# cristicbz/rust-doom

Hardware: NVIDIA H100
Metric: frames/sec at 1920x1080 (palette-index bit-exact) (higher is better)
Workload: dtype u8

## Files before the change

rust-doom_b200/csrc/b2d_kernels.cu:

```cuda
#include "b2d_kernels.cuh"

namespace b2d {

namespace {

constexpr unsigned kFull = 0xFFFFFFFFu;

constexpr int kMaskWords = 128;
constexpr int kStackDepth = 128;

constexpr uint32_t kVisBit = 1u << 25, kSolidBit = 1u << 24;
__device__ __forceinline__ uint32_t pack_range(int lo, int hi, uint32_t bits) {
    return (uint32_t)lo | ((uint32_t)hi << 12) | bits;
}
__device__ __forceinline__ int range_lo(uint32_t r) { return (int)(r & 0xFFFu); }
__device__ __forceinline__ int range_hi(uint32_t r) { return (int)((r >> 12) & 0xFFFu); }

__device__ __forceinline__ uint32_t word_bits(int w, int lo, int hi) {
    int a = max(lo, w * 32), b = min(hi, w * 32 + 31);
    if (a > b) return 0u;
    uint32_t m = 0xFFFFFFFFu >> (31 - (b - w * 32));
    return m & (0xFFFFFFFFu << (a - w * 32));
}

// ... 409 lines not shown
    uint8_t *p8 = c.fb + (size_t)y0 * Wc;
    uint32_t *p32 = kRgba ? c.rgba + (size_t)y0 * Wc : nullptr;
#pragma unroll 2
    for (int y = y0; y < y1; y++, p8 += Wc, p32 += Wc) {
        const uint32_t r = sc.skyrow[y];
        put_px<kRgba>(c, p8, p32, y >= ya && y < yb, __ldg(px + (inter ? (r >> 2) * w4 + (r & 3u) : r * T.w)));
    }
}

template <bool kRgba, int kW>
__device__ __forceinline__ void draw_plane_warp(const RasterCtx &c, const FrameConst &fc, const View &vw,
                                                int ya, int yb, int32_t h, int32_t flat, int lightb,
                                                bool visible) {
    const DeviceScene &sc = *c.sc;
    if (!__any_sync(kFull, ya < yb)) return;
    if (!visible) { fill_void_warp<kRgba, kW>(c, ya, yb); return; }
    if (flat == kFlatSky) { draw_sky_warp<kRgba, kW>(c, ya, yb); return; }
    if (flat < 0 || flat >= sc.nflats) { fill_void_warp<kRgba, kW>(c, ya, yb); return; }
    const uint64_t px_hi = reinterpret_cast<uint64_t>(sc.lit_flats) & 0xFFFFFFFF00000000ull;
    const uint32_t habs = plane_habs(h, fc.pose.z);
    bool act = ya < yb;
    int y0 = __reduce_min_sync(kFull, act ? ya : 0x7FFFFFFF);
    int y1 = __reduce_max_sync(kFull, act ? yb : 0);
    const int full_lo = __reduce_max_sync(kFull, act ? ya : 0x7FFFFFFF);
    const int full_hi = __reduce_min_sync(kFull, act ? yb : 0);
    const int Wc = kW ? kW : c.W;
    uint8_t *p8 = c.fb + (size_t)y0 * Wc;
    uint32_t *p32 = kRgba ? c.rgba + (size_t)y0 * Wc : nullptr;
    const uint32_t bu = (uint32_t)fc.pose.x << 10, bv = (uint32_t)fc.pose.y << 10;
    const uint32_t ax = (uint32_t)c.dir.ax, ay = (uint32_t)c.dir.ay;
    for (int yc = y0; yc < y1; yc += 32) {
        int yy = yc + c.lane;
        if (yy < y1) {
            const PlaneRow pr = plane_row(habs, sc.yslope[yy]);
            c.rowz[c.lane] = make_uint2(pr.z8q, (sc.lit_flat_stride >> 6) * (uint32_t)light_row(lightb, pr.z8) + 64u * (uint32_t)flat);
        }
        __syncwarp();
        const int rows = min(32, y1 - yc);
        int j = 0;
        for (; j + kBatch <= rows; j += kBatch, p8 += (size_t)kBatch * Wc, p32 += (size_t)kBatch * Wc) {
            uint32_t v[kBatch];
#pragma unroll
            for (int k = 0; k < kBatch; k++) {
                const uint2 rz = c.rowz[j + k];
                v[k] = __ldg(reinterpret_cast<const uint8_t *>(px_hi | flat_offset(rz.y, bu + rz.x * ax, bv + rz.x * ay)));
            }
            const int y = yc + j;
            store_batch<kRgba, kW>(c, p8, p32, v, y, ya, yb, y >= full_lo && y + kBatch <= full_hi);
        }
        for (; j < rows; j++, p8 += Wc, p32 += Wc) {
            const uint2 rz = c.rowz[j];
            const int y = yc + j;
            put_px<kRgba>(c, p8, p32, y >= ya && y < yb,
                          __ldg(reinterpret_cast<const uint8_t *>(px_hi | flat_offset(rz.y, bu + rz.x * ax, bv + rz.x * ay))));
        }
        __syncwarp();
    }
}

template <bool kRgba, int kW, int R>
__device__ __forceinline__ void wall_fast_loop(const RasterCtx &c, const uint8_t *plq, uint32_t w4, uint32_t nq, uint32_t q,
                                               uint32_t acc, uint32_t ts29, int y0, int y1, int ya, int yb,
                                               int full_lo, int full_hi) {
    const int Wc = kW ? kW : c.W;
    uint8_t *p8 = c.fb + (size_t)y0 * Wc;
    uint32_t *p32 = kRgba ? c.rgba + (size_t)y0 * Wc : nullptr;
    asm("" : "+l"(plq));
#pragma unroll 1
    for (int y = y0; y < y1; y += R, p8 += (size_t)R * Wc, p32 += (size_t)R * Wc) {
        const uint32_t q1 = q + 1u == nq ? 0u : q + 1u;
        const uint32_t w0 = __ldg(reinterpret_cast<const uint32_t *>(plq + (size_t)q * w4));
        const uint32_t w1 = __ldg(reinterpret_cast<const uint32_t *>(plq + (size_t)q1 * w4));
        if (y >= full_lo && y + R <= full_hi) {
#pragma unroll
            for (int k = 0; k < R; k++) {
                uint32_t v = pick_byte(w0, w1, wall_sel(acc, ts29, (uint32_t)k));
                if (kRgba) v &= 0xFFu;
                put_px<kRgba>(c, p8 + (size_t)k * Wc, kRgba ? p32 + (size_t)k * Wc : nullptr, true, v);
            }
        } else {
            const uint32_t m = row_mask(y, ya, yb, R);
#pragma unroll
            for (int k = 0; k < R; k++) {
                uint32_t v = pick_byte(w0, w1, wall_sel(acc, ts29, (uint32_t)k));
                if (kRgba) v &= 0xFFu;
                put_px<kRgba>(c, p8 + (size_t)k * Wc, kRgba ? p32 + (size_t)k * Wc : nullptr, (m >> k) & 1u, v);
            }
        }
        wall_advance(acc, q, ts29, (uint32_t)R, nq);
    }
}

template <bool kRgba, int kW>
__device__ __forceinline__ void draw_wall_warp(const RasterCtx &c, const FrameConst &fc, int ya, int yb,
                                               int32_t tex, int32_t tA, int32_t hA, int32_t ucol,
                                               int32_t iscale, int row) {
    const DeviceScene &sc = *c.sc;
    if (!__any_sync(kFull, ya < yb)) return;
    if (tex < 0 || tex >= sc.ntex) { fill_void_warp<kRgba, kW>(c, ya, yb); return; }
    const TexRec T = sc.tex[tex];
    bool act = ya < yb;
    const uint32_t col = (uint32_t)floormod32(ucol, (int32_t)T.w);
    const uint8_t *pl = sc.lit_texels + (size_t)row * sc.lit_texel_stride + T.texel_off;
    const uint32_t tstep = (uint32_t)(iscale >> 4);
    int y0 = __reduce_min_sync(kFull, act ? ya : 0x7FFFFFFF);
    int y1 = __reduce_max_sync(kFull, act ? yb : 0);
    const int full_lo = __reduce_max_sync(kFull, act ? ya : 0x7FFFFFFF);
    const int full_hi = __reduce_min_sync(kFull, act ? yb : 0);
    uint32_t t = (uint32_t)wall_tbase(tA, hA, fc.pose.z, c.H, iscale) + (uint32_t)y0 * tstep;
    const int Wc = kW ? kW : c.W;
    uint8_t *p8 = c.fb + (size_t)y0 * Wc;
    uint32_t *p32 = kRgba ? c.rgba + (size_t)y0 * Wc : nullptr;
    if (tex_interleaved(T) && T.h >= 8u) {
        const uint32_t ts = act ? tstep : 0u;
        const bool f16 = __all_sync(kFull, ts <= kWallFast16);
        if (f16 || __all_sync(kFull, ts <= kWallFast8)) {
            const uint32_t tt = act ? t : 0u;
            const uint32_t r0 = wall_row((int32_t)tt, T.h, T.hmagic, T.hbias);
            const uint8_t *plq = pl + 4u * col;
            if (f16) wall_fast_loop<kRgba, kW, 16>(c, plq, 4u * T.w, T.h >> 2, r0 >> 2, wall_acc29(tt, r0), ts << 13, y0, y1, ya, yb, full_lo, full_hi);
            else wall_fast_loop<kRgba, kW, 8>(c, plq, 4u * T.w, T.h >> 2, r0 >> 2, wall_acc29(tt, r0), ts << 13, y0, y1, ya, yb, full_lo, full_hi);
            return;
        }
    }
    if (tex_interleaved(T)) {
        const uint32_t colb = 4u * col, w4 = 4u * T.w;
        for (int y = y0; y < y1; y += kBatch, p8 += (size_t)kBatch * Wc, p32 += (size_t)kBatch * Wc, t += (uint32_t)kBatch * tstep) {
            const uint32_t r0 = wall_row((int32_t)t, T.h, T.hmagic, T.hbias);
            const uint32_t acc = wall_acc(t, r0);
            const uint32_t b7 = (acc + 7u * tstep) >> 16;
            uint32_t v[kBatch];
            if (__all_sync(kFull, b7 < 8u)) {
                const uint32_t q0 = r0 >> 2, q1 = next_quad(q0, T.h);
                const uint32_t w0 = __ldg(reinterpret_cast<const uint32_t *>(pl + (q0 * w4 + colb)));
                const uint32_t w1 = __ldg(reinterpret_cast<const uint32_t *>(pl + (q1 * w4 + colb)));
#pragma unroll
                for (int k = 0; k < kBatch; k++) {
                    v[k] = pick_byte(w0, w1, (acc + (uint32_t)k * tstep) >> 16);
                    if (kRgba) v[k] &= 0xFFu;
                }
            } else {
                const uint32_t t4 = t + 4u * tstep;
                const uint32_t r4 = wall_row((int32_t)t4, T.h, T.hmagic, T.hbias);
                const uint32_t acc4 = wall_acc(t4, r4);
                if (__all_sync(kFull, ((acc + 3u * tstep) >> 16) < 8u && ((acc4 + 3u * tstep) >> 16) < 8u)) {
                    const uint32_t q0 = r0 >> 2, q4 = r4 >> 2;
                    const uint32_t a0 = __ldg(reinterpret_cast<const uint32_t *>(pl + (q0 * w4 + colb)));
                    const uint32_t a1 = __ldg(reinterpret_cast<const uint32_t *>(pl + (next_quad(q0, T.h) * w4 + colb)));
                    const uint32_t b0 = __ldg(reinterpret_cast<const uint32_t *>(pl + (q4 * w4 + colb)));
                    const uint32_t b1 = __ldg(reinterpret_cast<const uint32_t *>(pl + (next_quad(q4, T.h) * w4 + colb)));
#pragma unroll
                    for (int k = 0; k < 4; k++) {
                        v[k] = pick_byte(a0, a1, (acc + (uint32_t)k * tstep) >> 16);
                        v[k + 4] = pick_byte(b0, b1, (acc4 + (uint32_t)k * tstep) >> 16);
                        if (kRgba) { v[k] &= 0xFFu; v[k + 4] &= 0xFFu; }
                    }
                } else {
#pragma unroll
                    for (int k = 0; k < kBatch; k++) {
                        const uint32_t rk = wall_row((int32_t)(t + (uint32_t)k * tstep), T.h, T.hmagic, T.hbias);
                        v[k] = __ldg(pl + ((rk >> 2) * w4 + colb + (rk & 3u)));
                    }
                }
            }
            store_batch<kRgba, kW>(c, p8, p32, v, y, ya, yb, y >= full_lo && y + kBatch <= full_hi);
        }
    } else {
        const uint8_t *px = pl + col;
#pragma unroll 1
        for (int y = y0; y < y1; y++, p8 += Wc, p32 += Wc, t += tstep)
            put_px<kRgba>(c, p8, p32, y >= ya && y < yb, __ldg(px + wall_row((int32_t)t, T.h, T.hmagic, T.hbias) * T.w));
    }
}

__device__ __forceinline__ uint32_t *masked_entry(const DeviceScene &sc, const uint32_t *chunks, int e) {
    return sc.masked_list + ((size_t)chunks[e / kMaskedChunk] * kMaskedChunk + (size_t)(e % kMaskedChunk)) * 33u;
}
__device__ __forceinline__ uint32_t *masked_push(const DeviceScene &sc, uint32_t *chunks, int &mcount, int lane) {
    bool ok = mcount < sc.masked_cap;
    if (ok && mcount % kMaskedChunk == 0) {
        uint32_t id = 0;
        if (lane == 0) id = atomicAdd(sc.masked_counter, 1u);
        id = __shfl_sync(kFull, id, 0);
        ok = id < sc.masked_chunks;
        if (ok && lane == 0) chunks[mcount / kMaskedChunk] = id;
        __syncwarp();
    }
    if (!ok) {
        if (lane == 0) atomicOr(sc.status_flag, kStatusMaskedFull);
        return nullptr;
    }
    return masked_entry(sc, chunks, mcount++);
}

template <bool kRgba, int kW, bool kStates, bool kLevels>
__device__ __noinline__ void masked_pass(const DeviceScene &sc, const View &vw, int32_t pose_z, uint8_t *fb,
                                         uint32_t *rgba, uint32_t pal_s, int x, int lane,
                                         const SegFrame *wl, const uint32_t *chunks, int count) {
    RasterCtx c;
    c.sc = &sc; c.pal_s = pal_s; c.fb = fb; c.rgba = rgba;
    c.W = vw.W; c.H = vw.H; c.x = x; c.lane = lane;
    const int Wc = kW ? kW : c.W;
    for (int e = count - 1; e >= 0; e--) {
        const uint32_t *ml = masked_entry(sc, chunks, e);
        const uint32_t k = ml[0];
        const uint32_t packed = ml[1 + c.lane];
        int ya = (int)(packed & 0xFFFFu), yb = (int)(packed >> 16);
        const SegFrame sf = wl[k];
        int32_t tex, tA, hA, ucol = 0, iscale = 1, row = 0;
        if (is_sprite_entry(sf)) {
            SpriteFrame sp;
            const SpriteRec P = sc.sprites[entry_sprite(sf, sp)];
            if (P.tex < 0 || P.tex >= sc.ntex) continue;
            const int32_t sw = (int32_t)sc.tex[P.tex].w, sh = (int32_t)sc.tex[P.tex].h;
            const int64_t scale = sprite_scale(vw, sp.cz);
            int32_t z8;
            scale_depth(vw, scale, iscale, z8);
            row = light_row_sprite(P.light, z8);
            tex = P.tex; tA = 0; hA = P.low + sh;
            if (ya < yb) {
                clip_rows(P.low + sh, P.low, row_scale(scale), pose_z, c.H, ya, yb);
                ucol = sprite_column(sp, vw, c.x, sw);
            }
        } else {
            const SegRec S = sc.segs[sf.seg];
            if (S.mid < 0 || S.mid >= sc.nmids) continue;
            const MidRec M = sc.mids[S.mid];
            tex = M.tex; tA = M.t_high; hA = M.high;
            ColumnEval ce = {0u, 1, 1, 0};
            if (ya < yb && column_eval(sf, vw, c.x, ce)) {
                clip_rows(M.high, M.low, ce.scale, pose_z, c.H, ya, yb);
                ucol = wall_column(S.uoff, S.len_q12, ce.s24);
                iscale = ce.iscale;
                row = light_row(S.light, ce.z8);
            } else {
                ya = yb = 0;
            }
        }
        if (tex < 0 || tex >= sc.ntex) continue;
        const TexRec T = sc.tex[tex];
        const bool act = ya < yb;
        int y0 = __reduce_min_sync(kFull, act ? ya : 0x7FFFFFFF);
        int y1 = __reduce_max_sync(kFull, act ? yb : 0);
        if (y0 >= y1) continue;
        const uint32_t col = (uint32_t)floormod32(ucol, (int32_t)T.w);
        const bool inter = tex_interleaved(T);
        const bool has_mask = T.mask_off != 0xFFFFFFFFu;
        const uint8_t *pl = sc.lit_texels + (size_t)row * sc.lit_texel_stride + T.texel_off;
        const uint8_t *pm = sc.lit_texels + (size_t)32 * sc.lit_texel_stride + T.texel_off;
        const uint32_t tstep = (uint32_t)(iscale >> 4);
        uint32_t t = (uint32_t)wall_tbase(tA, hA, pose_z, c.H, iscale) + (uint32_t)y0 * tstep;
        uint8_t *p8 = c.fb + (size_t)y0 * Wc;
        uint32_t *p32 = kRgba ? c.rgba + (size_t)y0 * Wc : nullptr;
        const uint32_t len = act ? (uint32_t)(yb - ya) : 0u;
        if (inter) {
            const uint32_t colb = 4u * col, w4 = 4u * T.w;
#pragma unroll 1
            for (int y = y0; y < y1; y += kBatch, p8 += (size_t)kBatch * Wc, p32 += (size_t)kBatch * Wc, t += (uint32_t)kBatch * tstep) {
                const uint32_t r0 = wall_row((int32_t)t, T.h, T.hmagic, T.hbias);
                const uint32_t acc = wall_acc(t, r0);
                const uint32_t d = (uint32_t)(y - ya);
                uint32_t v[kBatch], o[kBatch];
                if (__all_sync(kFull, ((acc + 7u * tstep) >> 16) < 8u)) {
                    const uint32_t o0 = (r0 >> 2) * w4 + colb, o1 = next_quad(r0 >> 2, T.h) * w4 + colb;
                    const uint32_t w0 = __ldg(reinterpret_cast<const uint32_t *>(pl + o0));
                    const uint32_t w1 = __ldg(reinterpret_cast<const uint32_t *>(pl + o1));
                    uint32_t m0 = 0x01010101u, m1 = 0x01010101u;
                    if (has_mask) {
                        m0 = __ldg(reinterpret_cast<const uint32_t *>(pm + o0));
                        m1 = __ldg(reinterpret_cast<const uint32_t *>(pm + o1));
                    }
#pragma unroll
                    for (int k = 0; k < kBatch; k++) {
                        const uint32_t bk = (acc + (uint32_t)k * tstep) >> 16;
                        v[k] = pick_byte(w0, w1, bk) & 0xFFu;
                        o[k] = pick_byte(m0, m1, bk) & 0xFFu;
                    }
                } else {
#pragma unroll
                    for (int k = 0; k < kBatch; k++) {
                        const uint32_t rk = wall_row((int32_t)(t + (uint32_t)k * tstep), T.h, T.hmagic, T.hbias);
                        const uint32_t off = (rk >> 2) * w4 + colb + (rk & 3u);
                        v[k] = __ldg(pl + off);
                        o[k] = has_mask ? (uint32_t)__ldg(pm + off) : 1u;
                    }
                }
#pragma unroll
                for (int k = 0; k < kBatch; k++)
                    put_px<kRgba>(c, p8 + (size_t)k * Wc, kRgba ? p32 + (size_t)k * Wc : nullptr, d + (uint32_t)k < len && o[k] != 0u, v[k]);
            }
        } else {
#pragma unroll 1
            for (int y = y0; y < y1; y++, p8 += Wc, p32 += Wc, t += tstep) {
                const uint32_t off = wall_row((int32_t)t, T.h, T.hmagic, T.hbias) * T.w + col;
                const bool on = (uint32_t)(y - ya) < len && (!has_mask || __ldg(pm + off) != 0);
                put_px<kRgba>(c, p8, p32, on, __ldg(pl + off));
            }
        }
    }
}

constexpr int kRasterWarps = 8;

template <bool kRgba, int kW, bool kMasked, bool kStates, bool kLevels>
__global__ void __launch_bounds__(32 * kRasterWarps, 16 / kRasterWarps)
b2d_raster_kernel(const __grid_constant__ DeviceScene sc, const __grid_constant__ View vw, const FrameConst *__restrict__ frames,
                  const SegFrame *__restrict__ work, int stride, int n, int strips,
                  uint8_t *__restrict__ index_fb, uint32_t *__restrict__ rgba_fb, const __grid_constant__ StateTables st,
                  const __grid_constant__ LevelTables lt) {
    __shared__ uint32_t s_pal[kRgba ? (kLevels ? 256 * kRasterWarps : 256) : 1];
    __shared__ uint2 s_rowz[kRasterWarps][32];
    __shared__ uint32_t s_chunks[kRasterWarps][kMasked ? kMaskedCapMax / kMaskedChunk : 1];
    if (kRgba && !kLevels) {
        for (int i = threadIdx.x; i < 256; i += blockDim.x) s_pal[i] = sc.palette[i];
        __syncthreads();
    }

    const int lane = threadIdx.x & 31;
    const long long gw = (long long)blockIdx.x * (blockDim.x >> 5) + (threadIdx.x >> 5);
    if (gw >= (long long)n * strips) return;
    const int frame = (int)(gw / strips), strip = (int)(gw % strips);
    const int W = kW ? kW : vw.W, H = vw.H;
    const int x0 = strip * 32, x = x0 + lane;
    const bool inside = x < W;

    const FrameConst fc = frames[frame];
    const DeviceScene *scp = &sc;
    if constexpr (kStates && !kLevels) {
        __shared__ DeviceScene s_sc[kRasterWarps];
        DeviceScene *d = &s_sc[threadIdx.x >> 5];
        const uint32_t *src = reinterpret_cast<const uint32_t *>(&sc);
        uint32_t *dst = reinterpret_cast<uint32_t *>(d);
        for (int i = lane; i < (int)(sizeof(DeviceScene) / 4); i += 32) dst[i] = src[i];
        __syncwarp();
        if (lane == 0) {
            const uint8_t *tb = st.base + (size_t)(uint32_t)fc.pad[0] * st.slot_bytes;
            d->tex = reinterpret_cast<const TexRec *>(tb);
            d->sectors = reinterpret_cast<const SectorRec *>(tb + st.off_sectors);
            d->segs = reinterpret_cast<const SegRec *>(tb + st.off_segs);
            d->sprites = reinterpret_cast<const SpriteRec *>(tb + st.off_sprites);
            d->mids = reinterpret_cast<const MidRec *>(tb + st.off_mids);
        }
        __syncwarp();
        scp = d;
    }
    if constexpr (kLevels) {
        __shared__ DeviceScene s_lv[kRasterWarps];
        DeviceScene *d = &s_lv[threadIdx.x >> 5];
        const DeviceScene *lsrc = lt.scenes + (uint32_t)fc.pad[1];
        const uint32_t *src = reinterpret_cast<const uint32_t *>(lsrc);
        uint32_t *dst = reinterpret_cast<uint32_t *>(d);
        for (int i = lane; i < (int)(sizeof(DeviceScene) / 4); i += 32) dst[i] = src[i];
        if (kRgba) {
            const uint32_t *pal = lsrc->palette;
            for (int i = lane; i < 256; i += 32) s_pal[256 * (threadIdx.x >> 5) + i] = pal[i];
        }
        __syncwarp();
        if constexpr (kStates) {
            if (lane == 0) {
                const TableSet t = lt.sets[(uint32_t)fc.pad[0]];
                d->tex = t.tex; d->sectors = t.sectors; d->segs = t.segs; d->sprites = t.sprites; d->mids = t.mids;
            }
            __syncwarp();
        }
        scp = d;
    }
    const DeviceScene &ts = *scp;
    const DeviceScene &ls = kLevels ? ts : sc;
    RasterCtx c;
    c.sc = &ts;
    c.pal_s = (uint32_t)__cvta_generic_to_shared(kLevels ? s_pal + 256 * (threadIdx.x >> 5) : s_pal);
    c.rowz = s_rowz[threadIdx.x >> 5];
    c.dir = plane_dir(fc, vw, inside ? x : 0, ls.invF);
    c.fb = index_fb + (size_t)frame * W * H + (inside ? x : 0);
    c.rgba = kRgba ? rgba_fb + (size_t)frame * W * H + (inside ? x : 0) : nullptr;
    c.W = W; c.H = H; c.x = x; c.lane = lane;
    c.skycol = 0;
    if (ls.sky_tex >= 0 && inside) c.skycol = umulhi32(sky_u32(x, vw, fc.pose.angle), ts.tex[ls.sky_tex].w);

    int ct = 0, cb = inside ? H : 0;
    uint32_t *chunks = s_chunks[threadIdx.x >> 5];
    asm("" : "+l"(chunks));
    const bool defer = kMasked && ls.masked_list != nullptr;
    int mcount = 0;
    const SegFrame *wl = work + (size_t)frame * stride;
    const int count = fc.count;
    bool done = false;

    for (int k0 = 0; k0 < count && !done; k0 += 32) {
        int k = k0 + lane;
        bool overlap = false;
        if (k < count) {
            int xlo = wl[k].xlo, xhi = wl[k].xhi;
            overlap = xhi >= x0 && xlo <= x0 + 31;
        }
        unsigned m = __ballot_sync(kFull, overlap);
        while (m) {
            int j = __ffs(m) - 1;
            m &= m - 1;
            if (!__any_sync(kFull, ct < cb)) { done = true; break; }
            const SegFrame sf = wl[k0 + j];
            bool in = inside && ct < cb && x >= sf.xlo && x <= sf.xhi;
            if (!__any_sync(kFull, in)) continue;
            if (is_sprite_entry(sf)) {
                if (defer) {
                    uint32_t *ml = masked_push(ls, chunks, mcount, lane);
                    if (ml) {
                        if (lane == 0) ml[0] = (uint32_t)(k0 + j);
                        ml[1 + lane] = in ? ((uint32_t)ct | ((uint32_t)cb << 16)) : 0u;
                    }
                }
                continue;
            }
            ColumnEval ce = {0u, 1, 1, 0};
            bool ok = in && column_eval(sf, vw, x, ce);
            if (!__any_sync(kFull, ok)) continue;

            const SegRec S = ts.segs[sf.seg];
            const SectorRec SF = ts.sectors[S.front];
            const int32_t fcl = SF.ceil, ffl = SF.floor;
            const bool two = S.flags & kSegTwoSided;
            const bool ceil_vis = plane_visible(true, fcl, SF.ceil_flat == kFlatSky, fc.pose.z);
            const bool floor_vis = plane_visible(false, ffl, SF.floor_flat == kFlatSky, fc.pose.z);

            WallRows wr = {ct, ct, ct, ct};
            int yend = ct, row = 0;
            int32_t ucol = 0;
            if (ok) {
                row = light_row(S.light, ce.z8);
                ucol = wall_column(S.uoff, S.len_q12, ce.s24);
                wr = wall_rows(fcl, ffl, two, S.otop, S.obot, ce.scale, fc.pose.z, H, ct, cb);
                yend = cb;
            }
#pragma unroll 1
            for (int pz = 0; pz < 2; pz++) {
                const bool top = pz == 0;
                draw_plane_warp<kRgba, kW>(c, fc, vw, ok ? (top ? ct : wr.y4) : 0, ok ? (top ? wr.y1 : yend) : 0,
                                                    top ? fcl : ffl, top ? SF.ceil_flat : SF.floor_flat, SF.light,
                                                    top ? ceil_vis : floor_vis);
            }
#pragma unroll 1
            for (int pw = 0; pw < 2; pw++) {
                const bool upper = pw == 0;
                if (!wall_piece(upper, two, fcl, ffl, S.otop, S.obot)) continue;
                draw_wall_warp<kRgba, kW>(c, fc, ok ? (upper ? wr.y1 : wr.y3) : 0, ok ? (upper ? wr.y2 : wr.y4) : 0,
                                                   upper ? S.texA : S.texB, upper ? S.tA : S.tB, upper ? S.hA : S.hB,
                                                   ucol, ce.iscale, row);
            }
            if (ok) wall_window(two, wr, H, ct, cb);
            if (defer && two && S.mid >= 0) {
                const bool keep = ok && wr.y2 < wr.y3;
                if (__any_sync(kFull, keep)) {
                    uint32_t *ml = masked_push(ls, chunks, mcount, lane);
                    if (ml) {
                        if (lane == 0) ml[0] = (uint32_t)(k0 + j);
                        ml[1 + lane] = keep ? ((uint32_t)wr.y2 | ((uint32_t)wr.y3 << 16)) : 0u;
                    }
                }
            }
        }
    }
    fill_void_warp<kRgba, kW>(c, inside ? ct : 0, inside ? cb : 0);
    if (kMasked && mcount > 0) {
        __syncwarp();
        masked_pass<kRgba, kW, kStates, kLevels>(ts, vw, fc.pose.z, c.fb, c.rgba, c.pal_s, x, lane, wl, chunks, mcount);
    }
}

__global__ void __launch_bounds__(256)
b2d_palette_kernel(const uint32_t *__restrict__ palette, const uint8_t *__restrict__ index,
                   uint32_t *__restrict__ rgba, size_t n_pixels) {
    __shared__ uint32_t s_pal[256];
    s_pal[threadIdx.x] = palette[threadIdx.x];
    __syncthreads();
    const bool aligned = ((reinterpret_cast<uintptr_t>(index) | reinterpret_cast<uintptr_t>(rgba)) & 15) == 0;
    const size_t nvec = aligned ? n_pixels / 16 : 0;
    const size_t stride = (size_t)gridDim.x * blockDim.x;
    for (size_t i = (size_t)blockIdx.x * blockDim.x + threadIdx.x; i < nvec; i += stride) {
        uint4 in = __ldcs(reinterpret_cast<const uint4 *>(index) + i);
        uint32_t wds[4] = {in.x, in.y, in.z, in.w};
        uint4 *out = reinterpret_cast<uint4 *>(rgba) + 4 * i;
#pragma unroll
        for (int q = 0; q < 4; q++) {
            uint4 o;
            o.x = s_pal[wds[q] & 0xFF];
            o.y = s_pal[(wds[q] >> 8) & 0xFF];
            o.z = s_pal[(wds[q] >> 16) & 0xFF];
            o.w = s_pal[wds[q] >> 24];
            __stcs(out + q, o);
        }
    }
    for (size_t p = nvec * 16 + (size_t)blockIdx.x * blockDim.x + threadIdx.x; p < n_pixels; p += stride)
        rgba[p] = s_pal[index[p]];
}

__global__ void __launch_bounds__(256)
b2d_palette_levels_kernel(const uint32_t *__restrict__ palettes, const uint32_t *__restrict__ tables,
                          const uint8_t *__restrict__ index, uint32_t *__restrict__ rgba, size_t npix, int parts) {
    __shared__ uint32_t s_pal[256];
    const size_t frame = blockIdx.x / parts;
    const int part = blockIdx.x % parts;
    s_pal[threadIdx.x] = palettes[(size_t)tables[frame] * 256 + threadIdx.x];
    __syncthreads();
    const uint8_t *in = index + frame * npix;
    uint32_t *out = rgba + frame * npix;
    const bool aligned = npix % 16 == 0 && ((reinterpret_cast<uintptr_t>(index) | reinterpret_cast<uintptr_t>(rgba)) & 15) == 0;
    const size_t n = aligned ? npix / 16 : npix;
    const size_t per = (n + parts - 1) / parts, lo = (size_t)part * per, hi = lo + per < n ? lo + per : n;
    if (aligned) {
        for (size_t i = lo + threadIdx.x; i < hi; i += blockDim.x) {
            const uint4 q = __ldcs(reinterpret_cast<const uint4 *>(in) + i);
            const uint32_t wds[4] = {q.x, q.y, q.z, q.w};
            uint4 *o4 = reinterpret_cast<uint4 *>(out) + 4 * i;
#pragma unroll
            for (int k = 0; k < 4; k++) {
                uint4 o;
                o.x = s_pal[wds[k] & 0xFF];
                o.y = s_pal[(wds[k] >> 8) & 0xFF];
                o.z = s_pal[(wds[k] >> 16) & 0xFF];
                o.w = s_pal[wds[k] >> 24];
                __stcs(o4 + k, o);
            }
        }
    } else {
        for (size_t p = lo + threadIdx.x; p < hi; p += blockDim.x) out[p] = s_pal[in[p]];
    }
}

constexpr int kResolveRgba = 0, kResolveRgb = 1, kResolvePlanar = 2, kResolveGray = 3;

template <int N>
__device__ __forceinline__ void store_run(uint8_t *dst, const uint32_t (&w)[(N + 3) / 4]) {
    const uintptr_t a = reinterpret_cast<uintptr_t>(dst);
    if constexpr (N % 16 == 0) {
        if ((a & 15) == 0) {
#pragma unroll
            for (int q = 0; q < N / 16; q++) __stcs(reinterpret_cast<uint4 *>(dst) + q, make_uint4(w[4 * q], w[4 * q + 1], w[4 * q + 2], w[4 * q + 3]));
            return;
        }
    }
    if constexpr (N % 8 == 0) {
        if ((a & 7) == 0) {
#pragma unroll
            for (int q = 0; q < N / 8; q++) __stcs(reinterpret_cast<uint2 *>(dst) + q, make_uint2(w[2 * q], w[2 * q + 1]));
            return;
        }
    }
    if constexpr (N % 4 == 0) {
        if ((a & 3) == 0) {
#pragma unroll
            for (int q = 0; q < N / 4; q++) __stcs(reinterpret_cast<unsigned int *>(dst) + q, w[q]);
            return;
        }
    }
    if constexpr (N % 2 == 0) {
        if ((a & 1) == 0) {
#pragma unroll
            for (int q = 0; q < N / 2; q++) reinterpret_cast<uint16_t *>(dst)[q] = (uint16_t)(w[q / 2] >> (16 * (q % 2)));
            return;
        }
    }
#pragma unroll
    for (int b = 0; b < N; b++) dst[b] = (uint8_t)(w[b / 4] >> (8 * (b % 4)));
}

template <int K, int FMT, int P>
__device__ __forceinline__ void resolve_emit(uint8_t *o, size_t opix, int OW, int y, int x0, const uint32_t (&acc0)[P],
                                             const uint32_t (&acc1)[P]) {
    constexpr uint32_t kk = K * K, half = K * K / 2;
    const size_t at = (size_t)y * OW + x0;
    if constexpr (FMT == kResolveGray) {
        uint32_t w[(P + 3) / 4] = {};
#pragma unroll
        for (int p = 0; p < P; p++) w[p / 4] |= ((acc0[p] + half) / kk) << (8 * (p % 4));
        store_run<P>(o + at, w);
    } else {
        uint32_t r[P], g[P], b[P];
#pragma unroll
        for (int p = 0; p < P; p++) {
            r[p] = ((acc0[p] & 0xFFFFu) + half) / kk;
            b[p] = ((acc0[p] >> 16) + half) / kk;
            g[p] = (acc1[p] + half) / kk;
        }
        if constexpr (FMT == kResolveRgba) {
            uint32_t w[P];
#pragma unroll
            for (int p = 0; p < P; p++) w[p] = r[p] | (g[p] << 8) | (b[p] << 16) | 0xFF000000u;
            store_run<4 * P>(o + 4 * at, w);
        } else if constexpr (FMT == kResolveRgb) {
            uint32_t w[(3 * P + 3) / 4] = {};
#pragma unroll
            for (int p = 0; p < P; p++) {
                w[(3 * p) / 4] |= r[p] << (8 * ((3 * p) % 4));
                w[(3 * p + 1) / 4] |= g[p] << (8 * ((3 * p + 1) % 4));
                w[(3 * p + 2) / 4] |= b[p] << (8 * ((3 * p + 2) % 4));
            }
            store_run<3 * P>(o + 3 * at, w);
        } else {
            uint32_t wr[(P + 3) / 4] = {}, wg[(P + 3) / 4] = {}, wb[(P + 3) / 4] = {};
#pragma unroll
            for (int p = 0; p < P; p++) {
                wr[p / 4] |= r[p] << (8 * (p % 4));
                wg[p / 4] |= g[p] << (8 * (p % 4));
                wb[p / 4] |= b[p] << (8 * (p % 4));
            }
            store_run<P>(o + at, wr);
            store_run<P>(o + opix + at, wg);
            store_run<P>(o + 2 * opix + at, wb);
        }
    }
}

template <int K, int FMT>
__global__ void __launch_bounds__(256)
b2d_resolve_kernel(const uint32_t *__restrict__ palettes, const uint32_t *__restrict__ tables, const uint8_t *__restrict__ index,
                   uint8_t *__restrict__ out, int W, int H, int parts, bool vec) {
    constexpr int P = K == 1 ? 16 : K == 2 ? 8 : K == 4 ? 4 : K == 6 ? 8 : K == 8 ? 2 : 16;
    constexpr int kBpp = FMT == kResolveRgba ? 4 : FMT == kResolveGray ? 1 : 3;
    __shared__ uint2 s_tab[256];
    const size_t frame = blockIdx.x / parts;
    const int part = blockIdx.x % parts;
    {
        const uint32_t c = palettes[(size_t)(tables ? tables[frame] : 0u) * 256 + threadIdx.x];
        const uint32_t R = c & 0xFF, G = (c >> 8) & 0xFF, B = (c >> 16) & 0xFF;
        s_tab[threadIdx.x] = FMT == kResolveGray ? make_uint2((77 * R + 150 * G + 29 * B + 128) >> 8, 0u) : make_uint2(R | (B << 16), G);
    }
    __syncthreads();
    const int OW = W / K, OH = H / K;
    const size_t opix = (size_t)OW * OH;
    const uint8_t *in = index + frame * (size_t)W * H;
    uint8_t *o = out + frame * opix * kBpp;
    if (vec) {
        const int groups = OW / P;
        const size_t n = (size_t)OH * groups, per = (n + parts - 1) / parts, lo = (size_t)part * per, hi = lo + per < n ? lo + per : n;
        for (size_t i = lo + threadIdx.x; i < hi; i += blockDim.x) {
            const int y = (int)(i / groups), x0 = (int)(i % groups) * P;
            const uint8_t *src = in + (size_t)y * K * W + (size_t)x0 * K;
            uint32_t acc0[P], acc1[P];
#pragma unroll
            for (int p = 0; p < P; p++) acc0[p] = acc1[p] = 0;
#pragma unroll
            for (int j = 0; j < K; j++) {
#pragma unroll
                for (int q = 0; q < P * K / 16; q++) {
                    const uint4 v = __ldcs(reinterpret_cast<const uint4 *>(src + (size_t)j * W) + q);
                    const uint32_t wds[4] = {v.x, v.y, v.z, v.w};
#pragma unroll
                    for (int b = 0; b < 16; b++) {
                        const uint2 t = s_tab[(wds[b / 4] >> (8 * (b % 4))) & 0xFF];
                        acc0[(16 * q + b) / K] += t.x;
                        if (FMT != kResolveGray) acc1[(16 * q + b) / K] += t.y;
                    }
                }
            }
            resolve_emit<K, FMT, P>(o, opix, OW, y, x0, acc0, acc1);
        }
    } else {
        const size_t n = opix, per = (n + parts - 1) / parts, lo = (size_t)part * per, hi = lo + per < n ? lo + per : n;
        for (size_t i = lo + threadIdx.x; i < hi; i += blockDim.x) {
            const int y = (int)(i / OW), x = (int)(i % OW);
            const uint8_t *src = in + (size_t)y * K * W + (size_t)x * K;
            uint32_t acc0[1] = {0}, acc1[1] = {0};
#pragma unroll
            for (int j = 0; j < K; j++) {
#pragma unroll
                for (int b = 0; b < K; b++) {
                    const uint2 t = s_tab[__ldcs(src + (size_t)j * W + b)];
                    acc0[0] += t.x;
                    if (FMT != kResolveGray) acc1[0] += t.y;
                }
            }
            resolve_emit<K, FMT, 1>(o, opix, OW, y, x, acc0, acc1);
        }
    }
}

}

size_t walk_smem_per_warp(const DeviceScene &sc) { return walk_layout(sc.nverts, sc.nsegs, sc.nnodes, sc.nss, sc.nsprites).total; }

static int device_sms() {
    int dev = 0, sms = 0;
    cudaGetDevice(&dev);
    cudaDeviceGetAttribute(&sms, cudaDevAttrMultiProcessorCount, dev);
    return sms > 0 ? sms : 1;
}

template <bool kStates, bool kLevels>
static cudaError_t walk_go(const BatchTables &t, size_t smem, const View &vw, const Pose *d_poses, int n, FrameConst *d_frames,
                           SegFrame *d_work, int stride, cudaStream_t stream, bool background) {
    if (n <= 0) return cudaSuccess;
    if (smem > 227 * 1024) return cudaErrorInvalidValue;
    if (smem > 48 * 1024) {
        cudaError_t e = cudaFuncSetAttribute(b2d_walk_kernel<kStates, kLevels>, cudaFuncAttributeMaxDynamicSharedMemorySize, (int)smem);
        if (e != cudaSuccess) return e;
    }
    const int sms = device_sms();
    const int blocks = (background && n > sms) ? sms : n, warps = 4;
    b2d_walk_kernel<kStates, kLevels><<<blocks, warps * 32, smem, stream>>>(t.scene, vw, d_poses, n, d_frames, d_work, stride,
                                                                            t.states, t.levels);
    return cudaGetLastError();
}

size_t walk_levels_static_smem() {
    static const size_t bytes = [] {
        cudaFuncAttributes a{}, b{};
        if (cudaFuncGetAttributes(&a, b2d_walk_kernel<false, true>) == cudaSuccess &&
            cudaFuncGetAttributes(&b, b2d_walk_kernel<true, true>) == cudaSuccess)
            return a.sharedSizeBytes > b.sharedSizeBytes ? a.sharedSizeBytes : b.sharedSizeBytes;
        cudaGetLastError();
        return sizeof(DeviceScene) + 16;
    }();
    return bytes;
}

cudaError_t launch_walk(const BatchTables &t, size_t levels_smem, const View &vw, const Pose *d_poses, int n,
                        FrameConst *d_frames, SegFrame *d_work, int stride, cudaStream_t stream, bool background) {
    if (t.per_level && levels_smem + walk_levels_static_smem() > kWalkSmemMax) return cudaErrorInvalidValue;
    const size_t smem = t.per_level ? levels_smem : walk_smem_per_warp(t.scene);
    auto go = t.per_level ? (t.per_frame ? walk_go<true, true> : walk_go<false, true>)
                          : (t.per_frame ? walk_go<true, false> : walk_go<false, false>);
    return go(t, smem, vw, d_poses, n, d_frames, d_work, stride, stream, background);
}

template <bool kStates, bool kLevels>
static cudaError_t raster_go(const BatchTables &t, bool masked, const View &vw, const FrameConst *d_frames,
                             const SegFrame *d_work, int stride, int n, uint8_t *d_index_fb, uint32_t *d_rgba,
                             cudaStream_t stream) {
    if (n <= 0) return cudaSuccess;
    const int strips = (vw.W + 31) / 32;
    const int nblocks = (int)(((long long)n * strips + kRasterWarps - 1) / kRasterWarps);
#define B2D_RASTER_GO(RGBA, KW) do { \
    if (masked) b2d_raster_kernel<RGBA, KW, true, kStates, kLevels><<<nblocks, 32 * kRasterWarps, 0, stream>>>(t.scene, vw, d_frames, d_work, stride, n, strips, d_index_fb, d_rgba, t.states, t.levels); \
    else b2d_raster_kernel<RGBA, KW, false, kStates, kLevels><<<nblocks, 32 * kRasterWarps, 0, stream>>>(t.scene, vw, d_frames, d_work, stride, n, strips, d_index_fb, d_rgba, t.states, t.levels); \
    } while (0)
    if (d_rgba) { if (vw.W == 1920) B2D_RASTER_GO(true, 1920); else B2D_RASTER_GO(true, 0); }
    else if (vw.W == 1920) B2D_RASTER_GO(false, 1920);
    else if (vw.W == 3840) B2D_RASTER_GO(false, 3840);
    else B2D_RASTER_GO(false, 0);
#undef B2D_RASTER_GO
    return cudaGetLastError();
}

cudaError_t launch_raster(const BatchTables &t, bool masked, const View &vw, const FrameConst *d_frames, const SegFrame *d_work,
                          int stride, int n, uint8_t *d_index_fb, uint32_t *d_rgba, cudaStream_t stream) {
    auto go = t.per_level ? (t.per_frame ? raster_go<true, true> : raster_go<false, true>)
                          : (t.per_frame ? raster_go<true, false> : raster_go<false, false>);
    return go(t, masked, vw, d_frames, d_work, stride, n, d_index_fb, d_rgba, stream);
}

namespace {
__global__ void __launch_bounds__(256)
b2d_prelight_kernel(const uint8_t *__restrict__ colormap, const uint8_t *__restrict__ src, uint8_t *__restrict__ dst,
                    size_t n, size_t stride) {
    __shared__ uint8_t cm[32 * 256];
    for (int i = threadIdx.x; i < 32 * 256; i += blockDim.x) cm[i] = colormap[i];
    __syncthreads();
    for (size_t i = (size_t)blockIdx.x * blockDim.x + threadIdx.x; i < n; i += (size_t)gridDim.x * blockDim.x) {
        const uint32_t t = src[i];
#pragma unroll 4
        for (int r = 0; r < 32; r++) dst[(size_t)r * stride + i] = cm[r * 256 + t];
    }
}
}

namespace {
__global__ void __launch_bounds__(256)
b2d_prelight_tex_kernel(const uint8_t *__restrict__ colormap, const uint8_t *__restrict__ texels,
// ... 133 lines not shown
```

Baseline: 526,300.

## Defer raster spans to a shared-memory queue drained by all warps in block

Plane, wall and void-fill spans are no longer drawn immediately by the warp that finds them. Each span is pushed as a record into a per-block shared-memory queue, and after a block barrier every warp pulls records through an atomic counter and draws them using the owning warp's per-lane context. The aim is to even out work across warps whose strips have very different depth complexity. In exchange it adds barriers, atomics and a large shared-memory footprint that may lower occupancy. It also packs iscale into 24 bits and routes the void fill through the plane path, either of which could break bit-exactness.

```diff
diff --git a/rust-doom_b200/csrc/b2d_kernels.cu b/rust-doom_b200/csrc/b2d_kernels.cu
--- a/rust-doom_b200/csrc/b2d_kernels.cu
+++ b/rust-doom_b200/csrc/b2d_kernels.cu
@@ -735,6 +735,39 @@
 
 constexpr int kRasterWarps = 8;
 
+constexpr uint32_t kQueueWords = 6144;
+constexpr uint32_t kQueueRecs = kQueueWords / 32;
+constexpr uint32_t kRecWall = 1u << 16, kRecVisible = 1u << 17;
+
+struct DrawQueue {
+    uint4 *head;
+    uint32_t *pool;
+    uint32_t *nrec, *nwords;
+};
+
+__device__ __forceinline__ bool queue_push(const DrawQueue &q, int lane, uint32_t meta, int32_t a, int32_t b, int32_t c,
+                                           int ya, int yb, int32_t ucol, uint32_t iscale_row) {
+    const bool act = ya < yb;
+    if (!__any_sync(kFull, act)) return true;
+    const bool wall = meta & kRecWall;
+    const uint32_t words = wall ? 96u : 32u;
+    uint32_t off = 0, i = kQueueRecs;
+    if (lane == 0) {
+        off = atomicAdd(q.nwords, words);
+        if (off + words <= kQueueWords) i = atomicAdd(q.nrec, 1u);
+    }
+    i = __shfl_sync(kFull, i, 0);
+    if (i >= kQueueRecs) return false;
+    off = __shfl_sync(kFull, off, 0);
+    q.pool[off + lane] = act ? (uint32_t)ya | ((uint32_t)yb << 16) : 0u;
+    if (wall) {
+        q.pool[off + 32 + lane] = (uint32_t)ucol;
+        q.pool[off + 64 + lane] = iscale_row;
+    }
+    if (lane == 0) q.head[i] = make_uint4(meta | off, (uint32_t)a, (uint32_t)b, (uint32_t)c);
+    return true;
+}
+
 template <bool kRgba, int kW, bool kMasked, bool kStates, bool kLevels>
 __global__ void __launch_bounds__(32 * kRasterWarps, 16 / kRasterWarps)
 b2d_raster_kernel(const __grid_constant__ DeviceScene sc, const __grid_constant__ View vw, const FrameConst *__restrict__ frames,
@@ -744,57 +777,68 @@
     __shared__ uint32_t s_pal[kRgba ? (kLevels ? 256 * kRasterWarps : 256) : 1];
     __shared__ uint2 s_rowz[kRasterWarps][32];
     __shared__ uint32_t s_chunks[kRasterWarps][kMasked ? kMaskedCapMax / kMaskedChunk : 1];
+    __shared__ int4 s_lanes[kRasterWarps][32];
+    __shared__ int s_frame[kRasterWarps];
+    __shared__ uint4 s_qhead[kQueueRecs];
+    __shared__ uint32_t s_qpool[kQueueWords];
+    __shared__ uint32_t s_qn[3];
+    __shared__ DeviceScene s_scn[kStates || kLevels ? kRasterWarps : 1];
+    if (threadIdx.x < 3) s_qn[threadIdx.x] = 0;
     if (kRgba && !kLevels) {
         for (int i = threadIdx.x; i < 256; i += blockDim.x) s_pal[i] = sc.palette[i];
-        __syncthreads();
-    }
-
-    const int lane = threadIdx.x & 31;
-    const long long gw = (long long)blockIdx.x * (blockDim.x >> 5) + (threadIdx.x >> 5);
-    if (gw >= (long long)n * strips) return;
-    const int frame = (int)(gw / strips), strip = (int)(gw % strips);
+    }
+    __syncthreads();
+
+    const int lane = threadIdx.x & 31, warp = threadIdx.x >> 5;
+    const long long gw = (long long)blockIdx.x * (blockDim.x >> 5) + warp;
+    const bool has_strip = gw < (long long)n * strips;
+    const int frame = has_strip ? (int)(gw / strips) : 0, strip = has_strip ? (int)(gw % strips) : 0;
     const int W = kW ? kW : vw.W, H = vw.H;
     const int x0 = strip * 32, x = x0 + lane;
-    const bool inside = x < W;
-
-    const FrameConst fc = frames[frame];
+    const bool inside = has_strip && x < W;
+    const DrawQueue q{s_qhead, s_qpool, &s_qn[0], &s_qn[1]};
+
+    FrameConst fc{};
+    if (has_strip) fc = frames[frame];
     const DeviceScene *scp = &sc;
     if constexpr (kStates && !kLevels) {
-        __shared__ DeviceScene s_sc[kRasterWarps];
-        DeviceScene *d = &s_sc[threadIdx.x >> 5];
-        const uint32_t *src = reinterpret_cast<const uint32_t *>(&sc);
-        uint32_t *dst = reinterpret_cast<uint32_t *>(d);
-        for (int i = lane; i < (int)(sizeof(DeviceScene) / 4); i += 32) dst[i] = src[i];
-        __syncwarp();
-        if (lane == 0) {
-            const uint8_t *tb = st.base + (size_t)(uint32_t)fc.pad[0] * st.slot_bytes;
-            d->tex = reinterpret_cast<const TexRec *>(tb);
-            d->sectors = reinterpret_cast<const SectorRec *>(tb + st.off_sectors);
-            d->segs = reinterpret_cast<const SegRec *>(tb + st.off_segs);
-            d->sprites = reinterpret_cast<const SpriteRec *>(tb + st.off_sprites);
-            d->mids = reinterpret_cast<const MidRec *>(tb + st.off_mids);
-        }
-        __syncwarp();
+        DeviceScene *d = &s_scn[warp];
+        if (has_strip) {
+            const uint32_t *src = reinterpret_cast<const uint32_t *>(&sc);
+            uint32_t *dst = reinterpret_cast<uint32_t *>(d);
+            for (int i = lane; i < (int)(sizeof(DeviceScene) / 4); i += 32) dst[i] = src[i];
+            __syncwarp();
+            if (lane == 0) {
+                const uint8_t *tb = st.base + (size_t)(uint32_t)fc.pad[0] * st.slot_bytes;
+                d->tex = reinterpret_cast<const TexRec *>(tb);
+                d->sectors = reinterpret_cast<const SectorRec *>(tb + st.off_sectors);
+                d->segs = reinterpret_cast<const SegRec *>(tb + st.off_segs);
+                d->sprites = reinterpret_cast<const SpriteRec *>(tb + st.off_sprites);
+                d->mids = reinterpret_cast<const MidRec *>(tb + st.off_mids);
+            }
+            __syncwarp();
+        }
         scp = d;
     }
     if constexpr (kLevels) {
-        __shared__ DeviceScene s_lv[kRasterWarps];
-        DeviceScene *d = &s_lv[threadIdx.x >> 5];
-        const DeviceScene *lsrc = lt.scenes + (uint32_t)fc.pad[1];
-        const uint32_t *src = reinterpret_cast<const uint32_t *>(lsrc);
-        uint32_t *dst = reinterpret_cast<uint32_t *>(d);
-        for (int i = lane; i < (int)(sizeof(DeviceScene) / 4); i += 32) dst[i] = src[i];
-        if (kRgba) {
-            const uint32_t *pal = lsrc->palette;
-            for (int i = lane; i < 256; i += 32) s_pal[256 * (threadIdx.x >> 5) + i] = pal[i];
-        }
-        __syncwarp();
-        if constexpr (kStates) {
-            if (lane == 0) {
-                const TableSet t = lt.sets[(uint32_t)fc.pad[0]];
-                d->tex = t.tex; d->sectors = t.sectors; d->segs = t.segs; d->sprites = t.sprites; d->mids = t.mids;
+        DeviceScene *d = &s_scn[warp];
+        if (has_strip) {
+            const DeviceScene *lsrc = lt.scenes + (uint32_t)fc.pad[1];
+            const uint32_t *src = reinterpret_cast<const uint32_t *>(lsrc);
+            uint32_t *dst = reinterpret_cast<uint32_t *>(d);
+            for (int i = lane; i < (int)(sizeof(DeviceScene) / 4); i += 32) dst[i] = src[i];
+            if (kRgba) {
+                const uint32_t *pal = lsrc->palette;
+                for (int i = lane; i < 256; i += 32) s_pal[256 * warp + i] = pal[i];
             }
             __syncwarp();
+            if constexpr (kStates) {
+                if (lane == 0) {
+                    const TableSet t = lt.sets[(uint32_t)fc.pad[0]];
+                    d->tex = t.tex; d->sectors = t.sectors; d->segs = t.segs; d->sprites = t.sprites; d->mids = t.mids;
+                }
+                __syncwarp();
+            }
         }
         scp = d;
     }
@@ -802,22 +846,27 @@
     const DeviceScene &ls = kLevels ? ts : sc;
     RasterCtx c;
     c.sc = &ts;
-    c.pal_s = (uint32_t)__cvta_generic_to_shared(kLevels ? s_pal + 256 * (threadIdx.x >> 5) : s_pal);
-    c.rowz = s_rowz[threadIdx.x >> 5];
+    c.pal_s = (uint32_t)__cvta_generic_to_shared(kLevels ? s_pal + 256 * warp : s_pal);
+    c.rowz = s_rowz[warp];
+    c.W = W; c.H = H; c.x = x; c.lane = lane;
+    int mcount = 0;
+    uint32_t *chunks = s_chunks[warp];
+    asm("" : "+l"(chunks));
+    const SegFrame *wl = work + (size_t)frame * stride;
+
+    if (has_strip) {
     c.dir = plane_dir(fc, vw, inside ? x : 0, ls.invF);
     c.fb = index_fb + (size_t)frame * W * H + (inside ? x : 0);
     c.rgba = kRgba ? rgba_fb + (size_t)frame * W * H + (inside ? x : 0) : nullptr;
-    c.W = W; c.H = H; c.x = x; c.lane = lane;
     c.skycol = 0;
     if (ls.sky_tex >= 0 && inside) c.skycol = umulhi32(sky_u32(x, vw, fc.pose.angle), ts.tex[ls.sky_tex].w);
+    s_lanes[warp][lane] = make_int4(c.dir.ax, c.dir.ay, (int)c.skycol, inside ? x : 0);
+    if (lane == 0) s_frame[warp] = frame;
 
     int ct = 0, cb = inside ? H : 0;
-    uint32_t *chunks = s_chunks[threadIdx.x >> 5];
-    asm("" : "+l"(chunks));
     const bool defer = kMasked && ls.masked_list != nullptr;
-    int mcount = 0;
-    const SegFrame *wl = work + (size_t)frame * stride;
     const int count = fc.count;
+    const uint32_t owner = (uint32_t)warp << 18;
     bool done = false;
 
     for (int k0 = 0; k0 < count && !done; k0 += 32) {
@@ -868,17 +917,20 @@
 #pragma unroll 1
             for (int pz = 0; pz < 2; pz++) {
                 const bool top = pz == 0;
-                draw_plane_warp<kRgba, kW>(c, fc, vw, ok ? (top ? ct : wr.y4) : 0, ok ? (top ? wr.y1 : yend) : 0,
-                                                    top ? fcl : ffl, top ? SF.ceil_flat : SF.floor_flat, SF.light,
-                                                    top ? ceil_vis : floor_vis);
+                const int ya = ok ? (top ? ct : wr.y4) : 0, yb = ok ? (top ? wr.y1 : yend) : 0;
+                const int32_t h = top ? fcl : ffl, flat = top ? SF.ceil_flat : SF.floor_flat;
+                const bool vis = top ? ceil_vis : floor_vis;
+                if (!queue_push(q, lane, owner | (vis ? kRecVisible : 0u), h, flat, SF.light, ya, yb, 0, 0u))
+                    draw_plane_warp<kRgba, kW>(c, fc, vw, ya, yb, h, flat, SF.light, vis);
             }
 #pragma unroll 1
             for (int pw = 0; pw < 2; pw++) {
                 const bool upper = pw == 0;
                 if (!wall_piece(upper, two, fcl, ffl, S.otop, S.obot)) continue;
-                draw_wall_warp<kRgba, kW>(c, fc, ok ? (upper ? wr.y1 : wr.y3) : 0, ok ? (upper ? wr.y2 : wr.y4) : 0,
-                                                   upper ? S.texA : S.texB, upper ? S.tA : S.tB, upper ? S.hA : S.hB,
-                                                   ucol, ce.iscale, row);
+                const int ya = ok ? (upper ? wr.y1 : wr.y3) : 0, yb = ok ? (upper ? wr.y2 : wr.y4) : 0;
+                const int32_t tex = upper ? S.texA : S.texB, tA = upper ? S.tA : S.tB, hA = upper ? S.hA : S.hB;
+                if (!queue_push(q, lane, owner | kRecWall, tex, tA, hA, ya, yb, ucol, (uint32_t)ce.iscale | ((uint32_t)row << 24)))
+                    draw_wall_warp<kRgba, kW>(c, fc, ya, yb, tex, tA, hA, ucol, ce.iscale, row);
             }
             if (ok) wall_window(two, wr, H, ct, cb);
             if (defer && two && S.mid >= 0) {
@@ -893,10 +945,44 @@
             }
         }
     }
-    fill_void_warp<kRgba, kW>(c, inside ? ct : 0, inside ? cb : 0);
-    if (kMasked && mcount > 0) {
-        __syncwarp();
-        masked_pass<kRgba, kW, kStates, kLevels>(ts, vw, fc.pose.z, c.fb, c.rgba, c.pal_s, x, lane, wl, chunks, mcount);
+    if (!queue_push(q, lane, owner, 0, 0, 0, inside ? ct : 0, inside ? cb : 0, 0, 0u))
+        fill_void_warp<kRgba, kW>(c, inside ? ct : 0, inside ? cb : 0);
+    }
+
+    __syncthreads();
+    const uint32_t nrec = min(s_qn[0], kQueueRecs);
+    for (;;) {
+        uint32_t i = 0;
+        if (lane == 0) i = atomicAdd(&s_qn[2], 1u);
+        i = __shfl_sync(kFull, i, 0);
+        if (i >= nrec) break;
+        const uint4 hd = s_qhead[i];
+        const uint32_t off = hd.x & 0xFFFFu, o = hd.x >> 18;
+        const int4 ln = s_lanes[o][lane];
+        const int f = s_frame[o];
+        const FrameConst fo = frames[f];
+        RasterCtx d;
+        d.sc = kStates || kLevels ? &s_scn[o] : &sc;
+        d.pal_s = (uint32_t)__cvta_generic_to_shared(kLevels ? s_pal + 256 * o : s_pal);
+        d.rowz = s_rowz[warp];
+        d.dir = PlaneDir{ln.x, ln.y};
+        d.fb = index_fb + (size_t)f * W * H + ln.w;
+        d.rgba = kRgba ? rgba_fb + (size_t)f * W * H + ln.w : nullptr;
+        d.W = W; d.H = H; d.x = ln.w; d.lane = lane;
+        d.skycol = (uint32_t)ln.z;
+        const uint32_t win = s_qpool[off + lane];
+        const int ya = (int)(win & 0xFFFFu), yb = (int)(win >> 16);
+        if (hd.x & kRecWall) {
+            const uint32_t isr = s_qpool[off + 64 + lane];
+            draw_wall_warp<kRgba, kW>(d, fo, ya, yb, (int32_t)hd.y, (int32_t)hd.z, (int32_t)hd.w, (int32_t)s_qpool[off + 32 + lane],
+                                      (int32_t)(isr & 0xFFFFFFu), (int)(isr >> 24));
+        } else {
+            draw_plane_warp<kRgba, kW>(d, fo, vw, ya, yb, (int32_t)hd.y, (int32_t)hd.z, (int)hd.w, hd.x & kRecVisible);
+        }
+    }
+    if constexpr (kMasked) {
+        __syncthreads();
+        if (mcount > 0) masked_pass<kRgba, kW, kStates, kLevels>(ts, vw, fc.pose.z, c.fb, c.rgba, c.pal_s, x, lane, wl, chunks, mcount);
     }
 }
 
```

Result: faster. 550,100 (median of 6 runs) (+4.5%).
